# bowman-lab/enspara

Measured on AMD Instinct MI355X. Metric: frame x center RMSD pairs/sec in k-centers assign, higher is better.
Workload: dtype f32

## Files before the change

### enspara_amd/_lib.py

```python
import ctypes as C
import os

import numpy as np

HERE = os.path.dirname(os.path.abspath(__file__))
LIB_PATH = os.environ.get("ENSPARA_HIP_LIB",
                          os.path.join(HERE, "libenspara_hip.so"))

EK_TILE = 256
EK_OK, EK_EARG, EK_EHIP, EK_ESTATE, EK_ENOMEM = 0, -1, -2, -3, -4

SYMBOLS = [
    "ek_abi_version", "ek_last_error", "ek_device_count",
    "ek_ctx_create", "ek_ctx_destroy", "ek_ctx_sync", "ek_ctx_stream",
    "ek_load_frames", "ek_rmsd_to_center",
    "ek_state_reset", "ek_state_download", "ek_state_upload",
    "ek_record_bytes", "ek_local_candidate", "ek_own_record",
    "ek_kcenters_step", "ek_kcenters_run",
    "ek_history_download", "ek_history_reset",
    "ek_spec_candidates", "ek_round_candidates", "ek_quad_copy_ready",
    "ek_spec_begin", "ek_spec_round", "ek_spec_localmax",
    "ek_spec_apply", "ek_spec_round_end", "ek_spec_progress", "ek_spec_rounds",
    "ek_spec_chain_bytes", "ek_spec_chain_rows", "ek_spec_chain_max",
    "ek_spec_chain_apply", "ek_run_stats", "ek_ti_stats", "ek_view_stats",
    "ek_ms_setup", "ek_ms_mailbox", "ek_ms_connect", "ek_ms_begin", "ek_ms_local",
    "ek_ms_global", "ek_ms_end", "ek_ms_run", "ek_ms_state", "ek_ms_diag",
    "ek_assign_nearest",
    "ek_pam_begin", "ek_pam_count_members", "ek_pam_select_member",
    "ek_pam_propose", "ek_pam_propose_member", "ek_pam_commit",
    "ek_pam_count_members_batch", "ek_pam_select_members_batch",
    "ek_pam_prefetch", "ek_pam_propose_ex", "ek_pam_prefetch_stats",
    "ek_pam_prefetch_window", "ek_pam_prefetch_passes", "ek_pam_sparse_stats", "ek_pam_ahead_stats", "ek_pam_window_run", "ek_pam_sweep", "ek_np_choice_draws",
    "ek_pam_window_max",
    "ek_pam_prefetch_centers_window",
    "ek_centered_frames", "ek_pam_begin_table", "ek_pam_prefetch_centers",
    "ek_pam_propose_center",
    "ek_msm_counts", "ek_msm_counts_ctx", "ek_msm_row_normalize",
    "ek_msm_mle_prinz", "ek_msm_bace_prune", "ek_msm_bace_run",
    "ek_lu_solve", "ek_lu_set_timing", "ek_lu_last_timing",
# ... 30 lines not shown
EK_OPT_FUSED_ROUNDS = 10
EK_OPT_TRIANGLE = 11
EK_OPT_PAM_ONE_WORKGROUP = 12
EK_OPT_PAM_MAX_PAIRS = 13
EK_OPT_PAM_BOTH_SUMS = 14
EK_OPT_FINE_PICK = 15
EK_OPT_PAM_BOUNDS = 16
EK_OPT_PICK_CAP = 17
EK_OPT_SMALL_SHARDS = 18
EK_OPT_PAM_AHEAD = 19
EK_OPT_PAM_ZERO_COPY = 20
EK_OPT_PAM_PAIRS_MFMA = 21
EK_OPT_PASS_SWEEP = 22
EK_OPT_MS_TWO_PHASE = 23
EK_OPT_ACTIVE_VIEW = 24
OPTIONS = {k[7:].lower(): v for k, v in list(globals().items())
           if k.startswith("EK_OPT_")}


class HipLibraryMissing(RuntimeError):
    pass


class HipError(RuntimeError):
    pass


_lib = None


# ... 54 lines not shown
    L.ek_spec_round_end.argtypes = [vp, vp]
    L.ek_spec_progress.argtypes = [vp, i32p, i32p]
    L.ek_spec_rounds.argtypes = [vp, i32p]
    L.ek_run_stats.argtypes = [vp, i64p, i64p]
    L.ek_ms_setup.argtypes = [vp, i32, i32, C.POINTER(C.c_size_t)]
    L.ek_ms_mailbox.argtypes = [vp, C.POINTER(vp), C.POINTER(vp), vp, vp]
    L.ek_ms_connect.argtypes = [vp, i32, vp, vp, vp, vp]
    L.ek_ms_begin.argtypes = [vp, i32, i32]
    L.ek_ms_local.argtypes = [vp, C.c_double, vp]
    L.ek_ms_global.argtypes = [vp, C.c_double, vp]
    L.ek_ms_end.argtypes = [vp]
    L.ek_ms_state.argtypes = [vp, i32p, i32p, i32p]
    L.ek_ms_run.argtypes = [vp, i32, i32, C.c_double, i32p, i64p, f32p, f32p]
    L.ek_ti_stats.argtypes = [vp, i64p, i64p]
    L.ek_view_stats.argtypes = [vp, i64p]
    L.ek_assign_nearest.argtypes = [vp, f32p, i32]
    f64p = C.POINTER(C.c_double)
    L.ek_ms_diag.argtypes = [vp, i64p, f64p]
    L.ek_pam_begin.argtypes = [vp, i64p, i32]
    L.ek_pam_count_members.argtypes = [vp, i32, i64p]
    L.ek_pam_select_member.argtypes = [vp, i32, i64, i64p]
    L.ek_pam_propose.argtypes = [vp, i32, i64, f64p, f64p, i64p]
    L.ek_pam_propose_member.argtypes = [vp, i32, i64, i64p, f64p, f64p, i64p]
    L.ek_pam_commit.argtypes = [vp, C.c_int]
    L.ek_pam_count_members_batch.argtypes = [vp, i32, i32, i64p]
    L.ek_pam_select_members_batch.argtypes = [vp, i32, i32, i64p, i64p]
    L.ek_pam_prefetch.argtypes = [vp, i64p, i32]
    L.ek_pam_propose_ex.argtypes = [vp, i32, i64, i64, i32, i32, f64p, f64p,
                                    i64p, C.POINTER(C.c_uint32)]
    L.ek_pam_prefetch_stats.argtypes = [vp, i64p, i64p]
# ... 123 lines not shown
```

### enspara_amd/csrc/ek_api.hip

```cpp
#include "ek_ctx.h"
#include "ek_view.h"
#include <cmath>
#include <mutex>
#include "ek_qcp.h"

static thread_local char g_err[512] = "";

int ek_set_error(int code, const char *fmt, ...)
{
    va_list ap;
    va_start(ap, fmt);
    vsnprintf(g_err, sizeof(g_err), fmt, ap);
    va_end(ap);
    return code;
}
void ek_ctx_msm_view(ek_ctx *c, int *device, int64_t *n, const int32_t **assign,
                     hipStream_t *stream, void ***scratch_slot)
{
    *device = c->device;
    *n = c->loaded ? c->n : -1;
    *assign = c->assign;
    *stream = c->stream;
    *scratch_slot = &c->msm_scratch;
}
// ... 556 lines not shown
            return ek_fail(EK_EARG, "ek_set_option: maxima per 64 frames for the pick 0 or 1");
        c->fine_pick = value;
        return EK_OK;
    case EK_OPT_MS_TWO_PHASE:
        if (value != 0 && value != 1)
            return ek_fail(EK_EARG, "ek_set_option: headers first in the mailbox rounds 0 or 1");
        c->ms_two_phase = value;
        return EK_OK;
    case EK_OPT_PASS_SWEEP:
        if (value < 0 || value > 2)
            return ek_fail(EK_EARG, "ek_set_option: per-prefix maxima in the pass 0, 1 "
                                    "(by the shard's size) or 2 (always)");
        c->pass_sweep = value;
        return EK_OK;
    case EK_OPT_ACTIVE_VIEW:
        if (value < 0 || value > 2)
            return ek_fail(EK_EARG, "ek_set_option: active view 0 (never), 1 (by the "
                                    "policy) or 2 (forced)");
        c->active_view = value;
        return EK_OK;
    case EK_OPT_ASSIGN_KERNEL:
        if (value < 0 || value > 3)
            return ek_fail(EK_EARG, "ek_set_option: assign variant 0..3");
        c->assign_variant = value;
        return EK_OK;
    default:
        return ek_fail(EK_EARG, "ek_set_option: unknown key %d", key);
    }
}

extern "C" int ek_get_option(ek_ctx *c, int32_t key, int32_t *value)
{
    if (!c || !value)
        return ek_fail(EK_EARG, "ek_get_option: NULL argument");
// ... 9 lines not shown
    case EK_OPT_FUSED_ROUNDS: *value = c->fused; return EK_OK;
    case EK_OPT_TRIANGLE: *value = c->tri; return EK_OK;
    case EK_OPT_PAM_ONE_WORKGROUP: *value = c->pam_sparse; return EK_OK;
    case EK_OPT_PAM_MAX_PAIRS: *value = c->sp_max_pairs; return EK_OK;
    case EK_OPT_PAM_BOTH_SUMS: *value = c->sp_exact; return EK_OK;
    case EK_OPT_FINE_PICK: *value = c->fine_pick; return EK_OK;
    case EK_OPT_PASS_SWEEP: *value = c->pass_sweep; return EK_OK;
    case EK_OPT_MS_TWO_PHASE: *value = c->ms_two_phase; return EK_OK;
    case EK_OPT_PAM_BOUNDS: *value = c->pam_bounds; return EK_OK;
    case EK_OPT_PICK_CAP: *value = c->pick_cap; return EK_OK;
    case EK_OPT_SMALL_SHARDS: *value = c->ms_small; return EK_OK;
    case EK_OPT_PAM_AHEAD: *value = c->pam_spec; return EK_OK;
    case EK_OPT_PAM_ZERO_COPY: *value = c->pam_zero_copy; return EK_OK;
    case EK_OPT_PAM_PAIRS_MFMA: *value = ek_pam_pairs_form; return EK_OK;
    case EK_OPT_ACTIVE_VIEW: *value = c->active_view; return EK_OK;
    default:
        return ek_fail(EK_EARG, "ek_get_option: unknown key %d", key);
    }
}

extern "C" int ek_last_run_timing(ek_ctx *c, float *ms, int32_t *launches)
{
    if (!c)
        return ek_fail(EK_EARG, "NULL context");
    if (ms)
        *ms = c->last_ms;
    if (launches)
        *launches = c->last_launches;
    return EK_OK;
}
// ... 366 lines not shown
                              hipMemcpyDeviceToHost, c->stream));
    }
    EK_HIP(ek_wait(c));
    for (int32_t i = 0; i < count; ++i) {
        const bool ok = i < avail && h[i].set;
        if (center_index_out)
            center_index_out[i] = ok ? h[i].gidx : -1;
        if (center_dist_out)
            center_dist_out[i] = ok ? h[i].dist : 0.f;
    }
    if (n_done)
        *n_done = ctl.n_done;
    return EK_OK;
}

static constexpr double EK_VIEW_RHO = 0.75;
static constexpr double EK_VIEW_SHRINK = 0.8;
static constexpr int EK_VIEW_MIN_ROUNDS = 24;
static constexpr int EK_VIEW_BATCH = 16;
static constexpr double EK_VIEW_REL = 1e-3, EK_VIEW_ABS = 1e-3;

void ek_view_free(ek_ctx *c)
{
    (void)hipFree(c->v_aos);
    (void)hipFree(c->v_tiles);
    (void)hipFree(c->v_qtiles);
    (void)hipFree(c->v_G);
    (void)hipFree(c->v_dist);
    (void)hipFree(c->v_assign);
    (void)hipFree(c->v_act);
    (void)hipFree(c->v_blockcnt);
    (void)hipFree(c->v_blockoff);
    (void)hipFree(c->v_count);
    c->v_aos = c->v_tiles = c->v_qtiles = nullptr;
// ... 15 lines not shown
    const size_t nblk = ek_view_sel_blocks(std::max<int64_t>(c->n, 1));
    hipError_t e = hipSuccess;
#define EK_VALLOC(ptr, bytes)                                                  \
    if (e == hipSuccess)                                                       \
        e = ek_malloc_named(c, (void **)&(ptr), (bytes), #ptr);
    EK_VALLOC(c->v_aos, (size_t)cap * A3 * sizeof(float));
    EK_VALLOC(c->v_tiles, nt * A3 * EK_TILE * sizeof(float));
    EK_VALLOC(c->v_qtiles, ek_quad_tiles_bytes((int64_t)nt, c->A));
    EK_VALLOC(c->v_G, (size_t)cap * sizeof(double));
    EK_VALLOC(c->v_dist, (size_t)cap * sizeof(float));
    EK_VALLOC(c->v_assign, (size_t)cap * sizeof(int32_t));
    EK_VALLOC(c->v_act, (size_t)cap * sizeof(uint32_t));
    EK_VALLOC(c->v_blockcnt, nblk * sizeof(uint32_t));
    EK_VALLOC(c->v_blockoff, nblk * sizeof(uint32_t));
    EK_VALLOC(c->v_count, 2 * sizeof(uint32_t));
#undef EK_VALLOC
    if (e != hipSuccess) {
        (void)hipGetLastError();
        ek_view_free(c);
        if (e == hipErrorOutOfMemory) {
            c->view_nomem = true;
            return EK_ENOMEM;
        }
        EK_HIP(e);
    }
    c->view_cap = cap;
    return EK_OK;
}

struct EkStore {
    float *dist;
    int32_t *assign;
    const float *tiles, *qtiles, *aos;
    const double *G;
    int64_t n, n_pad;
};
struct EkViewRun {
    bool on = false;
    int64_t n = 0;
    int32_t label_lo = 0;
    double guard = 0.0;
};

static void ek_view_scatter_back(ek_ctx *c, EkViewRun &v)
{
    ek_launch_view_scatter(c->v_act, v.n, c->v_dist, c->v_assign, c->dist, c->assign,
                           c->hist, v.label_lo, c->hist_cap, c->ctl, c->goff, c->stream);
    v.on = false;
}

static int ek_run_rounds_in(ek_ctx *c, int Tmax, int32_t first_label,
                            int32_t max_new, double dist_cutoff, int32_t *n_added,
                            int64_t *center_index_out, float *center_dist_out,
                            float *final_maxdist, EkViewRun &view);

static int ek_run_rounds(ek_ctx *c, int Tmax, int32_t first_label,
                         int32_t max_new, double dist_cutoff, int32_t *n_added,
// ... 129 lines not shown
        R.dist = S.dist;
        R.assign = S.assign;
        R.n = S.n;
        R.n_pad = S.n_pad;
        R.tiles = S.tiles;
        R.qtiles = S.qtiles;
        R.aos = S.aos;
        R.G = S.G;
        R.sweep = (fused && (c->pass_sweep == 2 ||
                             (c->pass_sweep == 1 && S.n <= (int64_t)2048 * EK_TILE))) ? 1 : 0;
        R.cutoff = the_view ? std::max(dist_cutoff, view.guard) : dist_cutoff;
    };
    use_store(false);
    int view_mode = (c->state_exact && c->A >= 3 && fused && !c->tri && !c->view_nomem)
                        ? c->active_view : 0;
    bool view_skip = true;
    auto leave_view = [&](bool &pending_) {
        if (pending_) {
            ek_launch_round_flush(R, c->stream);
            pending_ = false;
        }
        ek_view_scatter_back(c, view);
        use_store(false);
    };
    bool pending = false;
    int ti_pause = 0, ti_pause_next = 2;
    bool masks_fresh = false;
    int cap = c->pick_cap > 0 ? c->pick_cap : 4;
    const bool cap_adaptive = c->pick_cap <= 0;
    bool cap_probing = false;
    int cap_wait = 0, cap_next_wait = 2, cap_form = 0;
// ... 1 lines not shown
    unsigned long long ti_seen[2] = {0, 0};
    EK_HIP(hipEventRecord(c->ev0, c->stream));
    EkCtl cr;
    memset(&cr, 0, sizeof(cr));
    cr.n_done = first_label;
    const int32_t goal = first_label + max_new;
    double per_round = 0.6 * form;
    int32_t rounds_before = 0;
    while (cr.n_done < goal) {
        const int32_t left = goal - cr.n_done;
        const bool one = form == 1;
        R.T = form;
        const bool masks = tri && fused && form >= 4 && ti_pause == 0;
        R.tmask = masks ? c->ti_tmask : nullptr;
        R.pick_cap = cap;
        if (view_mode && view_skip) {
            view_skip = false;
        } else if (view_mode && std::isfinite(cr.last_max)) {
            const double th = (EK_VIEW_RHO * (double)cr.last_max - EK_VIEW_ABS) /
                              (2.0 * (1.0 + EK_VIEW_REL));
            float theta = (float)th;
            if ((double)theta > th)
                theta = std::nextafterf(theta, 0.f);
            const bool forced = view_mode == 2;
            const int64_t want_cap =
                forced ? c->n : (int64_t)std::ceil(EK_VIEW_SHRINK * (double)c->n);
            if (theta > 0.f && ek_view_alloc(c, want_cap) == EK_OK) {
                uint32_t cnt[2] = {0, 0};
                ek_launch_view_select(S.dist, S.n, theta, c->v_blockcnt, nullptr, nullptr, 0,
                                      c->v_count, c->stream);
                if (view.on)
                    ek_launch_view_select(c->dist, c->n, theta, c->v_blockcnt, nullptr,
                                          nullptr, 0, c->v_count + 1, c->stream);
                EK_CHECK_LAUNCH();
                EK_HIP(hipMemcpyAsync(cnt, c->v_count, sizeof(cnt), hipMemcpyDeviceToHost,
                                      c->stream));
                EK_HIP(ek_wait(c));
                const int64_t est = (int64_t)cnt[0] +
                                    (view.on ? std::max<int64_t>(0, (int64_t)cnt[1] - view.n)
                                             : 0);
                const bool build =
                    forced ? est < c->n
                           : ((double)est <= EK_VIEW_SHRINK * (double)S.n &&
                              (double)left >= EK_VIEW_MIN_ROUNDS * std::max(per_round, 1.0));
                if (build) {
                    if (view.on) {
                        leave_view(pending);
                    } else if (pending) {
                        ek_launch_round_flush(R, c->stream);
                        pending = false;
                    }
                    uint32_t nv = 0;
                    ek_launch_view_select(c->dist, c->n, theta, c->v_blockcnt,
                                          c->v_blockoff, c->v_act, c->view_cap, c->v_count,
                                          c->stream);
                    EK_CHECK_LAUNCH();
                    EK_HIP(hipMemcpyAsync(&nv, c->v_count, sizeof(nv),
                                          hipMemcpyDeviceToHost, c->stream));
                    EK_HIP(ek_wait(c));
                    if (nv > 0 && (int64_t)nv < c->n && (int64_t)nv <= c->view_cap) {
                        view.n = nv;
                        view.label_lo = cr.n_done;
                        view.guard = 2.0 * (double)theta * (1.0 + EK_VIEW_REL) + EK_VIEW_ABS;
                        ek_launch_view_gather(c->v_act, view.n, c->A, c->aos, c->G, c->dist,
                                              c->assign, c->v_aos, c->v_tiles, c->v_G,
                                              c->v_dist, c->v_assign, c->stream);
                        if (c->qt_valid)
                            ek_launch_quad_tiles(c->v_tiles, (view.n + EK_TILE - 1) / EK_TILE,
                                                 c->A, c->v_qtiles, c->stream);
                        EK_CHECK_LAUNCH();
                        view.on = true;
                        use_store(true);
                        EK_HIP(hipMemsetAsync(c->vmask, 0,
                                              (size_t)(S.n_pad / EK_WAVE) * sizeof(uint32_t),
                                              c->stream));
                        c->view_stats[0]++;
                    }
                    held = -1;
                }
            } else if (theta > 0.f) {
                (void)hipGetLastError();
                view_mode = 0;
            }
        }
        if (held != form) {
            if (pending) {
                ek_launch_round_flush(R, c->stream);
                pending = false;
            } else if (held <= 1) {
                ek_launch_blockmax(S.dist, S.n, c->blockmax, c->stream);
            }
            if (one) {
                ek_launch_pick(c->blockmax, nb, S.dist, S.tiles, S.G, S.n,
                               c->A, c->goff, c->recsT, c->ctl, c->stream);
            } else if (fused) {
                ek_launch_round_chain(R, 1, c->stream);
                ek_launch_round_next(R, 1, c->stream);
                ek_launch_round_ti(R, goal, c->stream);
// ... 5 lines not shown
            }
            EK_CHECK_LAUNCH();
            if (held != form && !one)
                per_round = 0.6 * form;
            held = form;
        }
        const int32_t due = adaptive ? std::max(gap - since, 1) : left;
        int32_t batch;
        if (one)
            batch = std::min(left, probing ? 4 : std::min(due, 256));
        else if (probing)
            batch = 3;
        else
            batch = std::max(2, std::min(256, (int32_t)(std::min(left, due) /
                                                        per_round) + 1));
        if (view_mode == 2)
            batch = std::min(batch, 2);
        else if (view_mode && !one)
            batch = std::min(batch, EK_VIEW_BATCH);
        EK_HIP(hipEventRecord(c->evb0, c->stream));
        if (R.tmask && !masks_fresh) {
            ek_launch_round_ti(R, goal, c->stream);
            masks_fresh = true;
        }
        if (!R.tmask)
            masks_fresh = false;
        for (int32_t r = 0; r < batch; ++r) {
            if (one) {
                const int label = cr.n_done + r;
                const bool skip = tri && label >= 1;
                if (skip)
                    ek_launch_ti(S.aos, S.G, c->A, c->hist, label, c->goff,
                                 c->recsT, c->ti_D, S.dist, S.assign, S.n,
                                 c->ctl, c->ti_skip, c->ti_stats, c->stream);
// ... 51 lines not shown
                ek_launch_chain_apply(c->vecs, S.n, S.n_pad, S.dist, S.assign,
                                      c->plan, c->blockmax, c->stream);
            } else {
                for (int j = 1; j < form; ++j) {
                    ek_launch_localmax_check(c->blockmax, nb, c->goff, R.cutoff,
                                             c->plan, c->hist, c->ctl, c->stream);
                    ek_launch_apply(c->vecs, S.G, S.n, S.n_pad, c->A, S.dist,
                                    S.assign, c->plan, c->blockmax, c->stream);
                }
            }
            ek_launch_pickT(c->blockmax, nb, S.tiles, S.G, S.assign, c->A, form,
                            c->goff, c->recsT, c->ctl, c->top, c->stream);
            EK_CHECK_LAUNCH();
        }
        EK_HIP(hipEventRecord(c->evb1, c->stream));
        const int32_t before = cr.n_done;
        EK_HIP(hipMemcpyAsync(&cr, c->ctl, sizeof(cr), hipMemcpyDeviceToHost,
                              c->stream));
        unsigned long long ti_now[2] = {ti_seen[0], ti_seen[1]};
        if (R.tmask)
            EK_HIP(hipMemcpyAsync(ti_now, c->ti_stats, sizeof(ti_now),
                                  hipMemcpyDeviceToHost, c->stream));
        EK_HIP(ek_wait(c));
        if (R.tmask) {
            const unsigned long long looked = ti_now[0] - ti_seen[0],
                                     left = ti_now[1] - ti_seen[1];
            ti_seen[0] = ti_now[0];
            ti_seen[1] = ti_now[1];
            if (looked > 0 && left * 50 < looked) {
                ti_pause = ti_pause_next;
// ... 9 lines not shown
        rounds_before = cr.n_rounds;
        c->st_rounds[ek_form_slot(form)] += ran;
        c->st_centers[ek_form_slot(form)] += got;
        c->view_stats[1] += (int64_t)ran * S.n;
        c->view_stats[2] += (int64_t)ran * (c->n - S.n);
        if (view.on && cr.stopped) {
            if ((double)cr.last_max > dist_cutoff)
                c->view_stats[3]++;
            leave_view(pending);
            const int32_t zero = 0;
            EK_HIP(hipMemcpyAsync(&c->ctl->stopped, &zero, sizeof(zero),
                                  hipMemcpyHostToDevice, c->stream));
            EK_HIP(ek_wait(c));
            cr.stopped = 0;
            held = -1;
            view_skip = true;
            if (cr.n_done < goal)
                continue;
        }
        if (cr.stopped || cr.n_done >= goal)
            break;
        if (!one)
            per_round = std::max(1.0, (double)got / std::max(ran, 1));
        if (cap_adaptive && !one && fused && ran > 0 && !probing) {
            const double yield = (double)got / ((double)ran * form);
            if (cap_probing) {
                cap_probing = false;
                if (form == cap_form && yield > cap_yield_home + 0.1) {
                    cap_next_wait = 2;
                } else {
                    cap = cap == 4 ? 16 : 4;
// ... 174 lines not shown
    const int32_t added = std::max(0, ctl.n_done - first_label);
    c->last_launches = added;
    if (n_added)
        *n_added = added;
    if (final_maxdist)
        *final_maxdist = ctl.last_max;
    if (added > 0 && (center_index_out || center_dist_out)) {
        rc = ek_history_download(c, first_label, added, center_index_out,
                                 center_dist_out, nullptr);
        if (rc)
            return rc;
    }
    return EK_OK;
}

extern "C" int ek_view_stats(ek_ctx *c, int64_t *stats)
{
    if (!c || !stats)
        return ek_fail(EK_EARG, "ek_view_stats: NULL argument");
    for (int k = 0; k < 4; ++k)
        stats[k] = c->view_stats[k];
    return EK_OK;
}

extern "C" int ek_timing_begin(ek_ctx *c, int32_t sample_every,
                               int32_t max_samples)
{
    if (!c || sample_every < 1 || max_samples < 1)
        return ek_fail(EK_EARG, "ek_timing_begin: bad argument");
    EK_HIP(hipSetDevice(c->device));
// ... 289 lines not shown
```

### enspara_amd/csrc/ek_ctx.h

```cpp
#pragma once
#include "ek_common.h"
#include "ek_pam_sparse.h"

#include <stdarg.h>
#include <stdio.h>
#include <stdlib.h>
#include <string.h>

#include <algorithm>
#include <condition_variable>
#include <mutex>
#include <new>
#include <thread>
#include <vector>

void ek_msm_scratch_free(void *w);

#define EK_N_FORMS 5

int ek_set_error(int code, const char *fmt, ...);
#define ek_fail ek_set_error

#define EK_HIP(call)                                                           \
    do {                                                                       \
// ... 224 lines not shown
    uint32_t *vmask = nullptr;
    struct Guard { const char *name; unsigned char *at; };
    std::vector<Guard> guards;
    unsigned int *tick = nullptr;
    float *ctile = nullptr;
    double *ctrace = nullptr;
    int chain = 1;
    int64_t n_pad = 0;
    int32_t last_passes = 0;
    int adapt = 1;
    int64_t st_rounds[EK_N_FORMS] = {0, 0, 0, 0, 0};
    int64_t st_centers[EK_N_FORMS] = {0, 0, 0, 0, 0};
    hipEvent_t evb0 = nullptr, evb1 = nullptr;

    int active_view = 1;
    bool view_nomem = false;
    int64_t view_cap = 0;
    float *v_aos = nullptr, *v_tiles = nullptr, *v_qtiles = nullptr;
    double *v_G = nullptr;
    float *v_dist = nullptr;
    int32_t *v_assign = nullptr;
    uint32_t *v_act = nullptr;
    uint32_t *v_blockcnt = nullptr, *v_blockoff = nullptr;
    uint32_t *v_count = nullptr;
    int64_t view_stats[4] = {0, 0, 0, 0};

    EkMsState *ms = nullptr;
    unsigned char *ms_mbox = nullptr;
    uint32_t *ms_flags = nullptr;
    EkMsXchg ms_x;
// ... 62 lines not shown
```

### enspara_amd/csrc/ek_view.h

```cpp
#pragma once
#include "ek_common.h"

#define EK_VIEW_SEL 1024

static inline size_t ek_view_sel_blocks(int64_t n)
{
    return (size_t)((n + EK_VIEW_SEL - 1) / EK_VIEW_SEL);
}
void ek_launch_view_select(const float *dist, int64_t n, float theta, uint32_t *blockcnt,
                           uint32_t *blockoff, uint32_t *act, int64_t act_cap,
                           uint32_t *count, hipStream_t s);
void ek_launch_view_gather(const uint32_t *act, int64_t n_v, int A, const float *aos,
                           const double *G, const float *dist, const int32_t *assign,
                           float *aos_v, float *tiles_v, double *G_v, float *dist_v,
                           int32_t *assign_v, hipStream_t s);
void ek_launch_view_scatter(const uint32_t *act, int64_t n_v, const float *dist_v,
                            const int32_t *assign_v, float *dist, int32_t *assign,
                            EkHist *hist, int32_t label_lo, int32_t label_cap,
                            const EkCtl *ctl, int64_t goff, hipStream_t s);
```

### enspara_amd/csrc/ek_view.hip

```cpp
#include "ek_view.h"

#define EK_VIEW_FPT (EK_VIEW_SEL / EK_BLOCK)
static_assert(EK_VIEW_FPT == 4, "a thread reads its frames' distances as one float4");

static __device__ __forceinline__ bool ek_view_active(float d, float theta)
{
    return !(d <= theta);
}

static __device__ __forceinline__ unsigned ek_view_flags(const float *__restrict__ dist,
                                                         int64_t f0, int64_t n, float theta)
{
    unsigned m = 0;
    if (f0 + EK_VIEW_FPT <= n) {
        const float4 t = *(const float4 *)(dist + f0);
        m = (ek_view_active(t.x, theta) ? 1u : 0u) | (ek_view_active(t.y, theta) ? 2u : 0u) |
            (ek_view_active(t.z, theta) ? 4u : 0u) | (ek_view_active(t.w, theta) ? 8u : 0u);
    } else {
        for (int q = 0; q < EK_VIEW_FPT; ++q)
            if (f0 + q < n && ek_view_active(dist[f0 + q], theta))
                m |= 1u << q;
    }
    return m;
}
// ... 141 lines not shown
    }
}

void ek_launch_view_gather(const uint32_t *act, int64_t n_v, int A, const float *aos,
                           const double *G, const float *dist, const int32_t *assign,
                           float *aos_v, float *tiles_v, double *G_v, float *dist_v,
                           int32_t *assign_v, hipStream_t s)
{
    if (n_v <= 0)
        return;
    const unsigned tiles = (unsigned)((n_v + EK_TILE - 1) / EK_TILE);
    hipLaunchKernelGGL(ek_view_gather_kernel, dim3(tiles), dim3(EK_BLOCK), 0, s, act, n_v, A,
                       aos, G, dist, assign, aos_v, tiles_v, G_v, dist_v, assign_v);
}

__global__ void __launch_bounds__(EK_BLOCK)
ek_view_scatter_kernel(const uint32_t *__restrict__ act, int64_t n_v,
                       const float *__restrict__ dist_v,
                       const int32_t *__restrict__ assign_v, float *__restrict__ dist,
                       int32_t *__restrict__ assign, EkHist *__restrict__ hist,
                       int32_t label_lo, int32_t label_cap, const EkCtl *__restrict__ ctl,
                       int64_t goff)
{
    const int64_t p = (int64_t)blockIdx.x * EK_BLOCK + threadIdx.x;
    if (p < n_v) {
        const uint32_t f = act[p];
        dist[f] = dist_v[p];
        assign[f] = assign_v[p];
    }
    int32_t hi = ctl->n_done;
// ... 22 lines not shown
```

### enspara_amd/device.py

```python
import ctypes as C

import numpy as np

from . import _lib
from .exception import DataInvalid


def as_xyz(X):
    if hasattr(X, "xyz"):
        X = X.xyz
    elif hasattr(X, "_data") and hasattr(X, "lengths"):
        X = X._data
    X = np.asarray(X)
    if X.ndim == 2 and X.shape[1] == 3:
        X = X[None]
    if X.ndim != 3 or X.shape[2] != 3:
        raise DataInvalid(
            "RMSD clustering needs coordinates shaped (n_frames, n_atoms, 3); "
            "got %s" % (X.shape,))
    return np.ascontiguousarray(X, dtype=np.float32)


def _option_key(key):
    if isinstance(key, str):
# ... 443 lines not shown
        k = np.zeros(5, dtype=np.int64)
        _lib.check(self.lib.ek_run_stats(self._h, _lib.i64p(p), _lib.i64p(k)))
        return {T: (int(p[i]), int(k[i])) for i, T in enumerate((1, 4, 8, 16, 32))}

    def ti_stats(self):
        t, k = C.c_int64(), C.c_int64()
        _lib.check(self.lib.ek_ti_stats(self._h, C.byref(t), C.byref(k)))
        return t.value, k.value

    def view_stats(self):
        s = np.zeros(4, dtype=np.int64)
        _lib.check(self.lib.ek_view_stats(self._h, _lib.i64p(s)))
        return {"views": int(s[0]), "streamed": int(s[1]), "left_out": int(s[2]),
                "guard_exits": int(s[3])}

    def history(self, first, count):
        idx = np.empty(max(count, 1), dtype=np.int64)
        cd = np.empty(max(count, 1), dtype=np.float32)
        nd = C.c_int32()
        _lib.check(self.lib.ek_history_download(
            self._h, int(first), int(count), _lib.i64p(idx), _lib.f32p(cd),
            C.byref(nd)))
        return idx[:count], cd[:count], nd.value

    def reset_history(self):
        _lib.check(self.lib.ek_history_reset(self._h))

    def set_frames_per_lane(self, fpl):
        _lib.check(self.lib.ek_set_frames_per_lane(self._h, int(fpl)))

# ... 30 lines not shown
```

### include/enspara_hip.h

```cpp
#ifndef ENSPARA_HIP_H
#define ENSPARA_HIP_H

#include <stddef.h>
#include <stdint.h>

#ifdef __cplusplus
extern "C" {
#endif

#define EK_ABI_VERSION 1
#define EK_TILE 256

#define EK_OK 0
#define EK_EARG (-1)
#define EK_EHIP (-2)
#define EK_ESTATE (-3)
#define EK_ENOMEM (-4)

typedef struct ek_ctx ek_ctx;

int ek_abi_version(void);
const char *ek_last_error(void);
int ek_device_count(void);

// ... 51 lines not shown
                  const void *ipc_mbox, const void *ipc_flags);
int ek_reserve_centers(ek_ctx *ctx, int32_t n_centers);
int ek_ms_begin(ek_ctx *ctx, int32_t first_label, int32_t limit);
int ek_ms_local(ek_ctx *ctx, double dist_cutoff, void *message_out);
int ek_ms_global(ek_ctx *ctx, double dist_cutoff, const void *messages_all);
int ek_ms_end(ek_ctx *ctx);
int ek_ms_diag(ek_ctx *ctx, int64_t *counts, double *ms);
int ek_ms_state(ek_ctx *ctx, int32_t *mode, int32_t *exchanges, int32_t *err);
int ek_ms_run(ek_ctx *ctx, int32_t first_label, int32_t max_new,
              double dist_cutoff, int32_t *n_added, int64_t *center_index_out,
              float *center_dist_out, float *final_maxdist);
int ek_spec_rounds(ek_ctx *ctx, int32_t *rounds);
int ek_run_stats(ek_ctx *ctx, int64_t *passes, int64_t *centers);
int ek_ti_stats(ek_ctx *ctx, int64_t *tiles, int64_t *skipped);
int ek_view_stats(ek_ctx *ctx, int64_t *stats);

int ek_history_download(ek_ctx *ctx, int32_t first, int32_t count,
                        int64_t *center_index_out, float *center_dist_out,
                        int32_t *n_done);
int ek_history_reset(ek_ctx *ctx);

int ek_assign_nearest(ek_ctx *ctx, const float *centers_xyz,
                      int32_t n_centers);

int ek_pam_begin(ek_ctx *ctx, const int64_t *medoid_frames, int32_t n_medoids);
int ek_pam_count_members(ek_ctx *ctx, int32_t cid, int64_t *count);
int ek_pam_select_member(ek_ctx *ctx, int32_t cid, int64_t j,
                         int64_t *frame_index);
int ek_pam_propose(ek_ctx *ctx, int32_t cid, int64_t frame_index,
                   double *old_cost, double *new_cost, int64_t *n_ambiguous);
// ... 170 lines not shown
    EK_OPT_PASS_FORM = 9,
    EK_OPT_FUSED_ROUNDS = 10,
    EK_OPT_TRIANGLE = 11,
    EK_OPT_PAM_ONE_WORKGROUP = 12,
    EK_OPT_PAM_MAX_PAIRS = 13,
    EK_OPT_PAM_BOTH_SUMS = 14,
    EK_OPT_FINE_PICK = 15,
    EK_OPT_PAM_BOUNDS = 16,
    EK_OPT_PICK_CAP = 17,
    EK_OPT_SMALL_SHARDS = 18,
    EK_OPT_PAM_AHEAD = 19,
    EK_OPT_PAM_ZERO_COPY = 20,
    EK_OPT_PAM_PAIRS_MFMA = 21,
    EK_OPT_PASS_SWEEP = 22,
    EK_OPT_MS_TWO_PHASE = 23,
    EK_OPT_ACTIVE_VIEW = 24
};
int ek_set_option(ek_ctx *ctx, int32_t key, int32_t value);
int ek_get_option(ek_ctx *ctx, int32_t key, int32_t *value);
int ek_last_run_timing(ek_ctx *ctx, float *ms, int32_t *launches);

int ek_timing_begin(ek_ctx *ctx, int32_t sample_every, int32_t max_samples);
int ek_timing_end(ek_ctx *ctx, float *avg_ms, int32_t *n_samples);
int ek_timing_form(ek_ctx *ctx, int32_t *candidates);
int ek_hbm_copy_rate(int device, size_t bytes, double *gbytes_per_s);
int ek_qcp_probe(int device, const float *S, const double *Gx, const double *Gy,
                 int32_t n_atoms, const float *cur, int64_t m, float *full,
                 float *below, unsigned char *cert);

int ek_debug_guards(ek_ctx *ctx);

// ... 5 lines not shown
```

Measured before the change: 22.02 billion.

## Overlap active-view probe with rounds, fuse view build, add adaptive pause

The active-view count probe now runs as a device-side kernel queued after each batch of rounds. It reads last_max from the control block and its counts return with the existing control readback, so the separate blocking sync per probe goes away. The gather and quad-tile steps are fused into one build kernel, and plain tiles are rebuilt lazily from quad tiles only when a non-MFMA form needs them. A backoff pause skips probes and allows larger batches while the estimate shows little shrinkage. The change also adds tunable rho/ratio options, a poison mode and a layout-check validation entry point, at the cost of added complexity and slightly staler view decisions.

```diff
diff --git a/enspara_amd/_lib.py b/enspara_amd/_lib.py
--- a/enspara_amd/_lib.py
+++ b/enspara_amd/_lib.py
@@ -23,6 +23,7 @@
     "ek_spec_apply", "ek_spec_round_end", "ek_spec_progress", "ek_spec_rounds",
     "ek_spec_chain_bytes", "ek_spec_chain_rows", "ek_spec_chain_max",
     "ek_spec_chain_apply", "ek_run_stats", "ek_ti_stats", "ek_view_stats",
+    "ek_view_layout_check",
     "ek_ms_setup", "ek_ms_mailbox", "ek_ms_connect", "ek_ms_begin", "ek_ms_local",
     "ek_ms_global", "ek_ms_end", "ek_ms_run", "ek_ms_state", "ek_ms_diag",
     "ek_assign_nearest",
@@ -83,6 +84,8 @@
 EK_OPT_PASS_SWEEP = 22
 EK_OPT_MS_TWO_PHASE = 23
 EK_OPT_ACTIVE_VIEW = 24
+EK_OPT_VIEW_RHO = 25
+EK_OPT_VIEW_RATIO = 26
 OPTIONS = {k[7:].lower(): v for k, v in list(globals().items())
            if k.startswith("EK_OPT_")}
 
@@ -167,6 +170,7 @@
     L.ek_ms_run.argtypes = [vp, i32, i32, C.c_double, i32p, i64p, f32p, f32p]
     L.ek_ti_stats.argtypes = [vp, i64p, i64p]
     L.ek_view_stats.argtypes = [vp, i64p]
+    L.ek_view_layout_check.argtypes = [vp, f32, i64p]
     L.ek_assign_nearest.argtypes = [vp, f32p, i32]
     f64p = C.POINTER(C.c_double)
     L.ek_ms_diag.argtypes = [vp, i64p, f64p]
diff --git a/enspara_amd/csrc/ek_api.hip b/enspara_amd/csrc/ek_api.hip
--- a/enspara_amd/csrc/ek_api.hip
+++ b/enspara_amd/csrc/ek_api.hip
@@ -594,10 +594,22 @@
         c->pass_sweep = value;
         return EK_OK;
     case EK_OPT_ACTIVE_VIEW:
-        if (value < 0 || value > 2)
+        if (value < 0 || value > 3)
             return ek_fail(EK_EARG, "ek_set_option: active view 0 (never), 1 (by the "
-                                    "policy) or 2 (forced)");
+                                    "policy), 2 (forced) or 3 (forced, poisoned)");
         c->active_view = value;
+        return EK_OK;
+    case EK_OPT_VIEW_RHO:
+        if (value < 500 || value > 950)
+            return ek_fail(EK_EARG, "ek_set_option: active view's guard 500 .. 950 per "
+                                    "mille of the maximum");
+        c->view_rho = value;
+        return EK_OK;
+    case EK_OPT_VIEW_RATIO:
+        if (value < 500 || value > 950)
+            return ek_fail(EK_EARG, "ek_set_option: active view's rebuild ratio 500 .. "
+                                    "950 per mille of the frames streamed");
+        c->view_ratio = value;
         return EK_OK;
     case EK_OPT_ASSIGN_KERNEL:
         if (value < 0 || value > 3)
@@ -637,6 +649,8 @@
     case EK_OPT_PAM_ZERO_COPY: *value = c->pam_zero_copy; return EK_OK;
     case EK_OPT_PAM_PAIRS_MFMA: *value = ek_pam_pairs_form; return EK_OK;
     case EK_OPT_ACTIVE_VIEW: *value = c->active_view; return EK_OK;
+    case EK_OPT_VIEW_RHO: *value = c->view_rho; return EK_OK;
+    case EK_OPT_VIEW_RATIO: *value = c->view_ratio; return EK_OK;
     default:
         return ek_fail(EK_EARG, "ek_get_option: unknown key %d", key);
     }
@@ -1033,10 +1047,11 @@
     return EK_OK;
 }
 
-static constexpr double EK_VIEW_RHO = 0.75;
-static constexpr double EK_VIEW_SHRINK = 0.8;
 static constexpr int EK_VIEW_MIN_ROUNDS = 24;
 static constexpr int EK_VIEW_BATCH = 16;
+static constexpr double EK_VIEW_IDLE = 0.95;
+static constexpr int EK_VIEW_PAUSE_MAX = 8;
+static constexpr int EK_VIEW_PAUSED_BATCH = 4 * EK_VIEW_BATCH;
 static constexpr double EK_VIEW_REL = 1e-3, EK_VIEW_ABS = 1e-3;
 
 void ek_view_free(ek_ctx *c)
@@ -1082,6 +1097,8 @@
     EK_VALLOC(c->v_blockcnt, nblk * sizeof(uint32_t));
     EK_VALLOC(c->v_blockoff, nblk * sizeof(uint32_t));
     EK_VALLOC(c->v_count, 2 * sizeof(uint32_t));
+    if (e == hipSuccess)
+        e = hipMemsetAsync(c->v_count, 0, 2 * sizeof(uint32_t), c->stream);
 #undef EK_VALLOC
     if (e != hipSuccess) {
         (void)hipGetLastError();
@@ -1108,7 +1125,34 @@
     int64_t n = 0;
     int32_t label_lo = 0;
     double guard = 0.0;
+    bool tiles_valid = false;
 };
+
+static hipError_t ek_view_poison(ek_ctx *c)
+{
+    const size_t cap = (size_t)c->view_cap, nt = cap / EK_TILE, A3 = (size_t)3 * c->A;
+    hipError_t e = hipMemsetAsync(c->v_aos, 0xFF, cap * A3 * sizeof(float), c->stream);
+    if (e == hipSuccess)
+        e = hipMemsetAsync(c->v_tiles, 0xFF, nt * A3 * EK_TILE * sizeof(float), c->stream);
+    if (e == hipSuccess)
+        e = hipMemsetAsync(c->v_qtiles, 0xFF, ek_quad_tiles_bytes((int64_t)nt, c->A),
+                           c->stream);
+    if (e == hipSuccess)
+        e = hipMemsetAsync(c->v_G, 0xFF, cap * sizeof(double), c->stream);
+    if (e == hipSuccess)
+        e = hipMemsetAsync(c->v_dist, 0xFF, cap * sizeof(float), c->stream);
+    if (e == hipSuccess)
+        e = hipMemsetAsync(c->v_assign, 0xFF, cap * sizeof(int32_t), c->stream);
+    return e;
+}
+
+static bool ek_view_build(ek_ctx *c, int64_t n_v)
+{
+    ek_launch_view_build(c->v_act, n_v, c->A, c->qt_valid, c->aos, c->G, c->dist, c->assign,
+                         c->v_aos, c->qt_valid ? c->v_qtiles : c->v_tiles, c->v_G, c->v_dist,
+                         c->v_assign, c->stream);
+    return !c->qt_valid;
+}
 
 static void ek_view_scatter_back(ek_ctx *c, EkViewRun &v)
 {
@@ -1268,7 +1312,11 @@
     use_store(false);
     int view_mode = (c->state_exact && c->A >= 3 && fused && !c->tri && !c->view_nomem)
                         ? c->active_view : 0;
-    bool view_skip = true;
+    const bool forced = view_mode >= 2;
+    const double rho = c->view_rho / 1000.0, shrink = c->view_ratio / 1000.0;
+    bool looked = false;
+    uint32_t look_cnt[2] = {0, 0};
+    int look_pause = 0, look_pause_next = 1;
     auto leave_view = [&](bool &pending_) {
         if (pending_) {
             ek_launch_round_flush(R, c->stream);
@@ -1300,35 +1348,29 @@
         const bool masks = tri && fused && form >= 4 && ti_pause == 0;
         R.tmask = masks ? c->ti_tmask : nullptr;
         R.pick_cap = cap;
-        if (view_mode && view_skip) {
-            view_skip = false;
-        } else if (view_mode && std::isfinite(cr.last_max)) {
-            const double th = (EK_VIEW_RHO * (double)cr.last_max - EK_VIEW_ABS) /
+        if (view_mode && looked && std::isfinite(cr.last_max)) {
+            looked = false;
+            const double th = (rho * (double)cr.last_max - EK_VIEW_ABS) /
                               (2.0 * (1.0 + EK_VIEW_REL));
             float theta = (float)th;
             if ((double)theta > th)
                 theta = std::nextafterf(theta, 0.f);
-            const bool forced = view_mode == 2;
-            const int64_t want_cap =
-                forced ? c->n : (int64_t)std::ceil(EK_VIEW_SHRINK * (double)c->n);
-            if (theta > 0.f && ek_view_alloc(c, want_cap) == EK_OK) {
-                uint32_t cnt[2] = {0, 0};
-                ek_launch_view_select(S.dist, S.n, theta, c->v_blockcnt, nullptr, nullptr, 0,
-                                      c->v_count, c->stream);
-                if (view.on)
-                    ek_launch_view_select(c->dist, c->n, theta, c->v_blockcnt, nullptr,
-                                          nullptr, 0, c->v_count + 1, c->stream);
-                EK_CHECK_LAUNCH();
-                EK_HIP(hipMemcpyAsync(cnt, c->v_count, sizeof(cnt), hipMemcpyDeviceToHost,
-                                      c->stream));
-                EK_HIP(ek_wait(c));
-                const int64_t est = (int64_t)cnt[0] +
-                                    (view.on ? std::max<int64_t>(0, (int64_t)cnt[1] - view.n)
-                                             : 0);
+            if (theta > 0.f) {
+                const int64_t est =
+                    (int64_t)look_cnt[0] +
+                    (view.on ? std::max<int64_t>(0, (int64_t)look_cnt[1] - view.n) : 0);
                 const bool build =
                     forced ? est < c->n
-                           : ((double)est <= EK_VIEW_SHRINK * (double)S.n &&
+                           : ((double)est <= shrink * (double)S.n &&
                               (double)left >= EK_VIEW_MIN_ROUNDS * std::max(per_round, 1.0));
+                if (!forced) {
+                    if ((double)est > EK_VIEW_IDLE * (double)S.n) {
+                        look_pause = look_pause_next;
+                        look_pause_next = std::min(2 * look_pause_next, EK_VIEW_PAUSE_MAX);
+                    } else if (build || (double)est <= shrink * (double)S.n) {
+                        look_pause_next = 1;
+                    }
+                }
                 if (build) {
                     if (view.on) {
                         leave_view(pending);
@@ -1348,12 +1390,9 @@
                         view.n = nv;
                         view.label_lo = cr.n_done;
                         view.guard = 2.0 * (double)theta * (1.0 + EK_VIEW_REL) + EK_VIEW_ABS;
-                        ek_launch_view_gather(c->v_act, view.n, c->A, c->aos, c->G, c->dist,
-                                              c->assign, c->v_aos, c->v_tiles, c->v_G,
-                                              c->v_dist, c->v_assign, c->stream);
-                        if (c->qt_valid)
-                            ek_launch_quad_tiles(c->v_tiles, (view.n + EK_TILE - 1) / EK_TILE,
-                                                 c->A, c->v_qtiles, c->stream);
+                        if (view_mode == 3)
+                            EK_HIP(ek_view_poison(c));
+                        view.tiles_valid = ek_view_build(c, view.n);
                         EK_CHECK_LAUNCH();
                         view.on = true;
                         use_store(true);
@@ -1364,10 +1403,13 @@
                     }
                     held = -1;
                 }
-            } else if (theta > 0.f) {
-                (void)hipGetLastError();
-                view_mode = 0;
             }
+        }
+        looked = false;
+        if (view.on && !view.tiles_valid && form < 16) {
+            ek_launch_view_tiles(c->v_qtiles, S.n_pad / EK_TILE, c->A, c->v_tiles, c->stream);
+            EK_CHECK_LAUNCH();
+            view.tiles_valid = true;
         }
         if (held != form) {
             if (pending) {
@@ -1403,10 +1445,10 @@
         else
             batch = std::max(2, std::min(256, (int32_t)(std::min(left, due) /
                                                         per_round) + 1));
-        if (view_mode == 2)
+        if (forced)
             batch = std::min(batch, 2);
         else if (view_mode && !one)
-            batch = std::min(batch, EK_VIEW_BATCH);
+            batch = std::min(batch, look_pause > 0 ? EK_VIEW_PAUSED_BATCH : EK_VIEW_BATCH);
         EK_HIP(hipEventRecord(c->evb0, c->stream));
         if (R.tmask && !masks_fresh) {
             ek_launch_round_ti(R, goal, c->stream);
@@ -1488,6 +1530,27 @@
             EK_CHECK_LAUNCH();
         }
         EK_HIP(hipEventRecord(c->evb1, c->stream));
+        if (view_mode && look_pause > 0) {
+            --look_pause;
+        } else if (view_mode) {
+            const int64_t want_cap =
+                forced ? c->n : (int64_t)std::ceil(shrink * (double)c->n);
+            if (ek_view_alloc(c, want_cap) == EK_OK) {
+                EK_HIP(hipMemsetAsync(c->v_count, 0, sizeof(look_cnt), c->stream));
+                ek_launch_view_look(S.dist, S.n, c->ctl, rho, EK_VIEW_REL, EK_VIEW_ABS,
+                                    c->v_count, c->stream);
+                if (view.on)
+                    ek_launch_view_look(c->dist, c->n, c->ctl, rho, EK_VIEW_REL,
+                                        EK_VIEW_ABS, c->v_count + 1, c->stream);
+                EK_CHECK_LAUNCH();
+                EK_HIP(hipMemcpyAsync(look_cnt, c->v_count, sizeof(look_cnt),
+                                      hipMemcpyDeviceToHost, c->stream));
+                looked = true;
+            } else {
+                (void)hipGetLastError();
+                view_mode = 0;
+            }
+        }
         const int32_t before = cr.n_done;
         EK_HIP(hipMemcpyAsync(&cr, c->ctl, sizeof(cr), hipMemcpyDeviceToHost,
                               c->stream));
@@ -1527,7 +1590,7 @@
             EK_HIP(ek_wait(c));
             cr.stopped = 0;
             held = -1;
-            view_skip = true;
+            looked = false;
             if (cr.n_done < goal)
                 continue;
         }
@@ -1732,6 +1795,85 @@
     return EK_OK;
 }
 
+extern "C" int ek_view_layout_check(ek_ctx *c, float theta, int64_t *out)
+{
+    if (!c || !out)
+        return ek_fail(EK_EARG, "ek_view_layout_check: NULL argument");
+    if (!c->loaded || c->n <= 0)
+        return ek_fail(EK_ESTATE, "ek_view_layout_check: no frames loaded");
+    EK_HIP(hipSetDevice(c->device));
+    out[0] = out[1] = out[2] = out[3] = 0;
+    int rc = ek_view_alloc(c, c->n);
+    if (rc)
+        return rc;
+    uint32_t nv = 0;
+    ek_launch_view_select(c->dist, c->n, theta, c->v_blockcnt, c->v_blockoff, c->v_act,
+                          c->view_cap, c->v_count, c->stream);
+    EK_CHECK_LAUNCH();
+    EK_HIP(hipMemcpyAsync(&nv, c->v_count, sizeof(nv), hipMemcpyDeviceToHost, c->stream));
+    EK_HIP(ek_wait(c));
+    out[0] = nv;
+    if (nv == 0 || (int64_t)nv > c->view_cap)
+        return EK_OK;
+    const size_t nt = ((size_t)nv + EK_TILE - 1) / EK_TILE, A3 = (size_t)3 * c->A;
+    const size_t tile_words = nt * A3 * EK_TILE;
+    const size_t quad_bytes = ek_quad_tiles_bytes((int64_t)nt, c->A);
+    float *r_aos = nullptr, *r_tiles = nullptr, *r_qtiles = nullptr, *r_dist = nullptr;
+    double *r_G = nullptr;
+    int32_t *r_assign = nullptr;
+    unsigned long long *diff = nullptr, got[3] = {0, 0, 0};
+    hipError_t e = hipMalloc((void **)&r_aos, (size_t)nv * A3 * sizeof(float));
+    if (e == hipSuccess)
+        e = hipMalloc((void **)&r_tiles, tile_words * sizeof(float));
+    if (e == hipSuccess)
+        e = hipMalloc((void **)&r_qtiles, quad_bytes);
+    if (e == hipSuccess)
+        e = hipMalloc((void **)&r_G, (size_t)nv * sizeof(double));
+    if (e == hipSuccess)
+        e = hipMalloc((void **)&r_dist, (size_t)nv * sizeof(float));
+    if (e == hipSuccess)
+        e = hipMalloc((void **)&r_assign, (size_t)nv * sizeof(int32_t));
+    if (e == hipSuccess)
+        e = hipMalloc((void **)&diff, sizeof(got));
+    if (e == hipSuccess)
+        e = hipMemsetAsync(diff, 0, sizeof(got), c->stream);
+    if (e == hipSuccess)
+        e = ek_view_poison(c);
+    if (e == hipSuccess) {
+        ek_launch_view_gather(c->v_act, nv, c->A, c->aos, c->G, c->dist, c->assign, r_aos,
+                              r_tiles, r_G, r_dist, r_assign, c->stream);
+        ek_launch_quad_tiles(r_tiles, (int64_t)nt, c->A, r_qtiles, c->stream);
+        if (!ek_view_build(c, nv))
+            ek_launch_view_tiles(c->v_qtiles, (int64_t)nt, c->A, c->v_tiles, c->stream);
+        if (c->qt_valid)
+            ek_launch_view_diff(c->v_qtiles, r_qtiles, quad_bytes / 4, diff, c->stream);
+        ek_launch_view_diff(c->v_tiles, r_tiles, tile_words, diff + 1, c->stream);
+        ek_launch_view_diff(c->v_aos, r_aos, (size_t)nv * A3, diff + 2, c->stream);
+        ek_launch_view_diff(c->v_G, r_G, (size_t)nv * 2, diff + 2, c->stream);
+        ek_launch_view_diff(c->v_dist, r_dist, (size_t)nv, diff + 2, c->stream);
+        ek_launch_view_diff(c->v_assign, r_assign, (size_t)nv, diff + 2, c->stream);
+        e = hipGetLastError();
+    }
+    if (e == hipSuccess)
+        e = hipMemcpyAsync(got, diff, sizeof(got), hipMemcpyDeviceToHost, c->stream);
+    if (e == hipSuccess)
+        e = ek_wait(c);
+    else
+        (void)hipStreamSynchronize(c->stream);
+    (void)hipFree(r_aos);
+    (void)hipFree(r_tiles);
+    (void)hipFree(r_qtiles);
+    (void)hipFree(r_G);
+    (void)hipFree(r_dist);
+    (void)hipFree(r_assign);
+    (void)hipFree(diff);
+    EK_HIP(e);
+    out[1] = (int64_t)got[0];
+    out[2] = (int64_t)got[1];
+    out[3] = (int64_t)got[2];
+    return EK_OK;
+}
+
 extern "C" int ek_view_stats(ek_ctx *c, int64_t *stats)
 {
     if (!c || !stats)
diff --git a/enspara_amd/csrc/ek_ctx.h b/enspara_amd/csrc/ek_ctx.h
--- a/enspara_amd/csrc/ek_ctx.h
+++ b/enspara_amd/csrc/ek_ctx.h
@@ -262,6 +262,8 @@
     hipEvent_t evb0 = nullptr, evb1 = nullptr;
 
     int active_view = 1;
+    int view_rho = 750;
+    int view_ratio = 800;
     bool view_nomem = false;
     int64_t view_cap = 0;
     float *v_aos = nullptr, *v_tiles = nullptr, *v_qtiles = nullptr;
diff --git a/enspara_amd/csrc/ek_view.h b/enspara_amd/csrc/ek_view.h
--- a/enspara_amd/csrc/ek_view.h
+++ b/enspara_amd/csrc/ek_view.h
@@ -14,6 +14,16 @@
                            const double *G, const float *dist, const int32_t *assign,
                            float *aos_v, float *tiles_v, double *G_v, float *dist_v,
                            int32_t *assign_v, hipStream_t s);
+void ek_launch_view_build(const uint32_t *act, int64_t n_v, int A, bool quad, const float *aos,
+                          const double *G, const float *dist, const int32_t *assign,
+                          float *aos_v, float *out_v, double *G_v, float *dist_v,
+                          int32_t *assign_v, hipStream_t s);
+void ek_launch_view_tiles(const float *qtiles, int64_t n_tiles, int A, float *tiles,
+                          hipStream_t s);
+void ek_launch_view_look(const float *dist, int64_t n, const EkCtl *ctl, double rho, double rel,
+                         double abs_, uint32_t *count, hipStream_t s);
+void ek_launch_view_diff(const void *a, const void *b, size_t words,
+                         unsigned long long *count, hipStream_t s);
 void ek_launch_view_scatter(const uint32_t *act, int64_t n_v, const float *dist_v,
                             const int32_t *assign_v, float *dist, int32_t *assign,
                             EkHist *hist, int32_t label_lo, int32_t label_cap,
diff --git a/enspara_amd/csrc/ek_view.hip b/enspara_amd/csrc/ek_view.hip
--- a/enspara_amd/csrc/ek_view.hip
+++ b/enspara_amd/csrc/ek_view.hip
@@ -1,3 +1,4 @@
+#include <algorithm>
 #include "ek_view.h"
 
 #define EK_VIEW_FPT (EK_VIEW_SEL / EK_BLOCK)
@@ -179,6 +180,236 @@
                        aos, G, dist, assign, aos_v, tiles_v, G_v, dist_v, assign_v);
 }
 
+#define EK_VIEW_BROWS 64
+#define EK_VIEW_BCH 64
+#define EK_VIEW_BROWF (3 * EK_VIEW_BCH + 1)
+typedef float ek_view_v4f __attribute__((ext_vector_type(4)));
+
+template <int VEC> struct EkViewVec;
+template <> struct EkViewVec<4> { typedef ek_view_v4f T; };
+template <> struct EkViewVec<1> { typedef float T; };
+
+template <int VEC, bool QUAD>
+__global__ void __launch_bounds__(EK_BLOCK)
+ek_view_build_kernel(const uint32_t *__restrict__ act, int64_t n_v, int A,
+                     const float *__restrict__ aos, const double *__restrict__ G,
+                     const float *__restrict__ dist, const int32_t *__restrict__ assign,
+                     float *__restrict__ aos_v, float *__restrict__ out_v,
+                     double *__restrict__ G_v, float *__restrict__ dist_v,
+                     int32_t *__restrict__ assign_v)
+{
+    static_assert(EK_BLOCK == 256 && EK_TILE == 256 && EK_WAVE == 64,
+                  "four workgroups per tile of the view, one per wave of the pass");
+    typedef typename EkViewVec<VEC>::T vec_t;
+    constexpr int LPR = EK_VIEW_BCH / VEC;
+    constexpr int RPS = EK_BLOCK / LPR;
+    constexpr int SWEEPS = EK_VIEW_BROWS / RPS;
+    __shared__ float stage[EK_VIEW_BROWS * EK_VIEW_BROWF];
+    __shared__ uint32_t src[EK_VIEW_BROWS];
+    const int t = threadIdx.x;
+    const size_t tile = blockIdx.x >> 2;
+    const int qw = blockIdx.x & 3;
+    const int64_t p0 = (int64_t)tile * EK_TILE + EK_VIEW_BROWS * qw;
+    const int rows_here =
+        (int)(n_v - p0 >= EK_VIEW_BROWS ? EK_VIEW_BROWS : (n_v > p0 ? n_v - p0 : 0));
+    if (t < EK_VIEW_BROWS) {
+        const int64_t p = p0 + t;
+        const uint32_t f = t < rows_here ? act[p] : 0u;
+        src[t] = f;
+        if (t < rows_here) {
+            G_v[p] = G[f];
+            dist_v[p] = dist[f];
+            assign_v[p] = assign[f];
+        }
+    }
+    __syncthreads();
+    const size_t A3 = (size_t)3 * A;
+    const int NQ = (A + 3) / 4;
+    const int jl = t & (LPR - 1), r0 = t / LPR;
+    const int slot = t & 63, wv = t >> 6, qe = slot >> 4, qf = slot & 15;
+    for (int a0 = 0; a0 < A; a0 += EK_VIEW_BCH) {
+        const int w = 3 * ((A - a0 < EK_VIEW_BCH) ? (A - a0) : EK_VIEW_BCH);
+        const int we = w / VEC;
+        vec_t v[SWEEPS][3];
+#pragma unroll
+        for (int it = 0; it < SWEEPS; ++it) {
+            const int r = r0 + it * RPS;
+            const vec_t *s = (const vec_t *)(aos + (size_t)src[r] * A3 + 3 * a0);
+#pragma unroll
+            for (int m = 0; m < 3; ++m) {
+                const int j = jl + m * LPR;
+                if (r < rows_here && j < we)
+                    v[it][m] = s[j];
+            }
+        }
+#pragma unroll
+        for (int it = 0; it < SWEEPS; ++it) {
+            const int r = r0 + it * RPS;
+            vec_t *d = (vec_t *)(aos_v + (size_t)(p0 + r) * A3 + 3 * a0);
+            float *st = stage + r * EK_VIEW_BROWF;
+#pragma unroll
+            for (int m = 0; m < 3; ++m) {
+                const int j = jl + m * LPR;
+                if (r < rows_here && j < we) {
+                    d[j] = v[it][m];
+                    if constexpr (VEC == 4) {
+#pragma unroll
+                        for (int x = 0; x < 4; ++x)
+                            st[4 * j + x] = v[it][m][x];
+                    } else {
+                        st[j] = v[it][m];
+                    }
+                }
+            }
+        }
+        __syncthreads();
+        if constexpr (QUAD) {
+            ek_view_v4f *dst = (ek_view_v4f *)out_v + tile * (size_t)NQ * 3 * EK_TILE +
+                               EK_VIEW_BROWS * qw + slot;
+            for (int qq = wv; qq < EK_VIEW_BCH / 4; qq += EK_BLOCK / EK_WAVE) {
+                const int q = a0 / 4 + qq;
+                if (q >= NQ)
+                    break;
+                const bool atom = 4 * q + qe < A;
+#pragma unroll
+                for (int k = 0; k < 3; ++k) {
+                    ek_view_v4f o;
+#pragma unroll
+                    for (int g = 0; g < 4; ++g) {
+                        const int fr = 16 * g + qf;
+                        o[g] = (atom && fr < rows_here)
+                                   ? stage[fr * EK_VIEW_BROWF + 3 * (4 * qq + qe) + k] : 0.f;
+                    }
+                    dst[(size_t)(q * 3 + k) * EK_TILE] = o;
+                }
+            }
+        } else {
+            float *tp = out_v + tile * A3 * EK_TILE + EK_VIEW_BROWS * qw + slot;
+            const float *row = stage + slot * EK_VIEW_BROWF;
+            for (int j = wv; j < w; j += EK_BLOCK / EK_WAVE)
+                tp[(size_t)(3 * a0 + j) * EK_TILE] = slot < rows_here ? row[j] : 0.f;
+        }
+        __syncthreads();
+    }
+}
+
+void ek_launch_view_build(const uint32_t *act, int64_t n_v, int A, bool quad, const float *aos,
+                          const double *G, const float *dist, const int32_t *assign,
+                          float *aos_v, float *out_v, double *G_v, float *dist_v,
+                          int32_t *assign_v, hipStream_t s)
+{
+    if (n_v <= 0)
+        return;
+    const unsigned tiles = (unsigned)((n_v + EK_TILE - 1) / EK_TILE);
+#define EK_VIEW_BUILD(VEC, QUAD)                                                          \
+    hipLaunchKernelGGL((ek_view_build_kernel<VEC, QUAD>), dim3(4 * tiles), dim3(EK_BLOCK), 0, \
+                       s, act, n_v, A, aos, G, dist, assign, aos_v, out_v, G_v, dist_v,   \
+                       assign_v)
+    if (A % 4 == 0) {
+        if (quad)
+            EK_VIEW_BUILD(4, true);
+        else
+            EK_VIEW_BUILD(4, false);
+    } else {
+        if (quad)
+            EK_VIEW_BUILD(1, true);
+        else
+            EK_VIEW_BUILD(1, false);
+    }
+#undef EK_VIEW_BUILD
+}
+
+__global__ void __launch_bounds__(EK_BLOCK)
+ek_view_tiles_kernel(const float *__restrict__ qtiles, int A, int NQ,
+                     float *__restrict__ tiles)
+{
+    const int l = threadIdx.x;
+    const int w = l >> 6, e = (l >> 4) & 3, f16 = l & 15;
+    const size_t tile = blockIdx.x;
+    const ek_view_v4f *src = (const ek_view_v4f *)qtiles + tile * (size_t)NQ * 3 * EK_TILE + l;
+    float *dst = tiles + tile * 3 * (size_t)A * EK_TILE + 64 * w + f16;
+    for (int q = blockIdx.y; q < NQ; q += gridDim.y) {
+        const int a = 4 * q + e;
+        if (a >= A)
+            continue;
+#pragma unroll
+        for (int k = 0; k < 3; ++k) {
+            const ek_view_v4f v = src[(size_t)(q * 3 + k) * EK_TILE];
+#pragma unroll
+            for (int g = 0; g < 4; ++g)
+                dst[(size_t)(3 * a + k) * EK_TILE + 16 * g] = v[g];
+        }
+    }
+}
+
+void ek_launch_view_tiles(const float *qtiles, int64_t n_tiles, int A, float *tiles,
+                          hipStream_t s)
+{
+    if (n_tiles <= 0)
+        return;
+    const int NQ = (A + 3) / 4;
+    const unsigned gy = (unsigned)std::max<int64_t>(
+        1, std::min<int64_t>(NQ, 2048 / std::max<int64_t>(n_tiles, 1)));
+    hipLaunchKernelGGL(ek_view_tiles_kernel, dim3((unsigned)n_tiles, gy), dim3(EK_BLOCK), 0, s,
+                       qtiles, A, NQ, tiles);
+}
+
+#define EK_VIEW_LOOK_SEL (8 * EK_VIEW_SEL)
+__global__ void __launch_bounds__(EK_BLOCK)
+ek_view_look_kernel(const float *__restrict__ dist, int64_t n, const EkCtl *__restrict__ ctl,
+                    double rho, double rel, double abs_, uint32_t *__restrict__ count)
+{
+    __shared__ unsigned red[EK_BLOCK / EK_WAVE];
+    const double th = (rho * (double)ctl->last_max - abs_) / (2.0 * (1.0 + rel));
+    float theta = (float)th;
+    if ((double)theta > th && theta > 0.f)
+        theta = __uint_as_float(__float_as_uint(theta) - 1u);
+    unsigned mine = 0;
+#pragma unroll
+    for (int q = 0; q < EK_VIEW_LOOK_SEL / EK_VIEW_SEL; ++q) {
+        const int64_t f0 = (((int64_t)blockIdx.x * (EK_VIEW_LOOK_SEL / EK_VIEW_SEL) + q) *
+                                EK_BLOCK + threadIdx.x) * EK_VIEW_FPT;
+        mine += f0 < n ? (unsigned)__popc(ek_view_flags(dist, f0, n, theta)) : 0u;
+    }
+    unsigned total;
+    (void)ek_view_block_scan(mine, red, &total);
+    if (threadIdx.x == 0 && total)
+        atomicAdd(count, total);
+}
+
+void ek_launch_view_look(const float *dist, int64_t n, const EkCtl *ctl, double rho, double rel,
+                         double abs_, uint32_t *count, hipStream_t s)
+{
+    if (n <= 0)
+        return;
+    hipLaunchKernelGGL(ek_view_look_kernel,
+                       dim3((unsigned)((n + EK_VIEW_LOOK_SEL - 1) / EK_VIEW_LOOK_SEL)),
+                       dim3(EK_BLOCK), 0, s, dist, n, ctl, rho, rel, abs_, count);
+}
+
+__global__ void __launch_bounds__(EK_BLOCK)
+ek_view_diff_kernel(const uint32_t *__restrict__ a, const uint32_t *__restrict__ b, size_t n,
+                    unsigned long long *__restrict__ count)
+{
+    unsigned mine = 0;
+    for (size_t i = (size_t)blockIdx.x * EK_BLOCK + threadIdx.x; i < n;
+         i += (size_t)gridDim.x * EK_BLOCK)
+        mine += a[i] != b[i] ? 1u : 0u;
+    if (mine)
+        atomicAdd(count, (unsigned long long)mine);
+}
+
+void ek_launch_view_diff(const void *a, const void *b, size_t words,
+                         unsigned long long *count, hipStream_t s)
+{
+    if (words == 0)
+        return;
+    const unsigned blocks =
+        (unsigned)std::min<size_t>((words + EK_BLOCK - 1) / EK_BLOCK, (size_t)4096);
+    hipLaunchKernelGGL(ek_view_diff_kernel, dim3(blocks), dim3(EK_BLOCK), 0, s,
+                       (const uint32_t *)a, (const uint32_t *)b, words, count);
+}
+
 __global__ void __launch_bounds__(EK_BLOCK)
 ek_view_scatter_kernel(const uint32_t *__restrict__ act, int64_t n_v,
                        const float *__restrict__ dist_v,
diff --git a/enspara_amd/device.py b/enspara_amd/device.py
--- a/enspara_amd/device.py
+++ b/enspara_amd/device.py
@@ -481,6 +481,11 @@
         return {"views": int(s[0]), "streamed": int(s[1]), "left_out": int(s[2]),
                 "guard_exits": int(s[3])}
 
+    def view_layout_check(self, theta):
+        out = np.zeros(4, dtype=np.int64)
+        _lib.check(self.lib.ek_view_layout_check(self._h, float(theta), _lib.i64p(out)))
+        return tuple(int(v) for v in out)
+
     def history(self, first, count):
         idx = np.empty(max(count, 1), dtype=np.int64)
         cd = np.empty(max(count, 1), dtype=np.float32)
diff --git a/include/enspara_hip.h b/include/enspara_hip.h
--- a/include/enspara_hip.h
+++ b/include/enspara_hip.h
@@ -89,6 +89,7 @@
 int ek_run_stats(ek_ctx *ctx, int64_t *passes, int64_t *centers);
 int ek_ti_stats(ek_ctx *ctx, int64_t *tiles, int64_t *skipped);
 int ek_view_stats(ek_ctx *ctx, int64_t *stats);
+int ek_view_layout_check(ek_ctx *ctx, float theta, int64_t *out);
 
 int ek_history_download(ek_ctx *ctx, int32_t first, int32_t count,
                         int64_t *center_index_out, float *center_dist_out,
@@ -289,7 +290,9 @@
     EK_OPT_PAM_PAIRS_MFMA = 21,
     EK_OPT_PASS_SWEEP = 22,
     EK_OPT_MS_TWO_PHASE = 23,
-    EK_OPT_ACTIVE_VIEW = 24
+    EK_OPT_ACTIVE_VIEW = 24,
+    EK_OPT_VIEW_RHO = 25,
+    EK_OPT_VIEW_RATIO = 26
 };
 int ek_set_option(ek_ctx *ctx, int32_t key, int32_t value);
 int ek_get_option(ek_ctx *ctx, int32_t key, int32_t *value);
```

New measurement: 23.05 billion (median of 6 runs). 1.05x the previous value.
